# sag2021/ndsm

Hardware: AMD Instinct MI355X
Metric: fine-grid LUP/s (RB-GS smoother updates per second of V-cycle time, fp64) (higher is better)
Workload: dtype f64; 1 GPU; 512^3 vector-potential Ax component, one V-cycle + convergence metric per step (ms=5, 8 grids), config[2] of BASELINE.json; global_points=134217728, parallelism=single GPU

## Files before the change

ndsm_amd/csrc/smooth.hip:

```cpp
#include "common.hpp"

namespace ndsm {
void fused_metric_accumulate(bool on);
int launch_rbgs3_fused(const ndsmk_grid &g, const double *u, double *uout, const double *rhs, int max_sweeps,
                       bool force, int *sweeps_done, double *rout, int *res_done, const double *prev, int *met_done,
                       const ndsmk_xfer *px, const double *uc);
int fetch_fused_metric(double *h_out2);
int launch_mean_shift(double *u, int64_t n);
}

namespace {

__device__ __forceinline__ size_t lin3(int i, int j, int k, int nx, int ny) {
  return (size_t)i + (size_t)nx * ((size_t)j + (size_t)ny * (size_t)k);
}

__global__ __launch_bounds__(256) void rbgs3_color(double *__restrict__ u, const double *__restrict__ rhs,
                                                  ndsmk_grid g, int par) {
  const int nx = g.n[0], ny = g.n[1], nz = g.n[2];
  const int j = g.lb[1] + blockIdx.y * blockDim.y + threadIdx.y;
  const int k = g.lb[2] + blockIdx.z;
  if (j > g.ub[1]) return;
  const int kg = k + g.k0;
  const int i0 = g.lb[0] + ((((g.lb[0] + j + kg) & 1) != par) ? 1 : 0);
  const int i = i0 + 2 * (blockIdx.x * blockDim.x + threadIdx.x);
  if (i > g.ub[0]) return;
  int xl = i - 1, xh = i + 1, yl = j - 1, yh = j + 1, zl = k - 1, zh = k + 1;
  if (xl < 0) xl = 1;
  if (xh > nx - 1) xh = nx - 2;
  if (yl < 0) yl = 1;
  if (yh > ny - 1) yh = ny - 2;
  if (kg - 1 < 0) zl = k + 1;
  if (kg + 1 > g.nzg - 1) zh = k - 1;
  (void)nz;
  const double unew = (u[lin3(xh, j, k, nx, ny)] + u[lin3(xl, j, k, nx, ny)]) * g.w[0] +
                      (u[lin3(i, yh, k, nx, ny)] + u[lin3(i, yl, k, nx, ny)]) * g.w[1] +
                      (u[lin3(i, j, zh, nx, ny)] + u[lin3(i, j, zl, nx, ny)]) * g.w[2] -
                      (rhs ? rhs[lin3(i, j, k, nx, ny)] : 0.0);
  u[lin3(i, j, k, nx, ny)] = g.w1 * unew;
}

__global__ __launch_bounds__(1024) void rbgs3_small(double *__restrict__ u_g, const double *__restrict__ rhs_g,
                                                    ndsmk_grid g, int nsweeps) {
  __shared__ double u[4096], rhs[4096];
  const int nx = g.n[0], ny = g.n[1];
  const int n = nx * ny * g.n[2];
  for (int p = threadIdx.x; p < n; p += blockDim.x) {
    u[p] = u_g[p];
    rhs[p] = rhs_g ? rhs_g[p] : 0.0;
  }
  __syncthreads();
  const int mx = g.ub[0] - g.lb[0] + 1, my = g.ub[1] - g.lb[1] + 1, mz = g.ub[2] - g.lb[2] + 1;
  const int half = (mx + 1) / 2;
  const int total = half * my * mz;
  for (int sw = 0; sw < nsweeps; ++sw) {
    for (int pass = 0; pass < 2; ++pass) {
      const int par = (g.first_par + pass) & 1;
      for (int p = threadIdx.x; p < total; p += blockDim.x) {
        const int t = p % half, j = g.lb[1] + (p / half) % my, k = g.lb[2] + p / (half * my);
        const int i0 = g.lb[0] + ((((g.lb[0] + j + k) & 1) != par) ? 1 : 0);
        const int i = i0 + 2 * t;
        if (i > g.ub[0]) continue;
        int xl = i - 1, xh = i + 1, yl = j - 1, yh = j + 1, zl = k - 1, zh = k + 1;
        if (xl < 0) xl = 1;
        if (xh > nx - 1) xh = nx - 2;
        if (yl < 0) yl = 1;
        if (yh > ny - 1) yh = ny - 2;
        if (zl < 0) zl = 1;
        if (zh > g.n[2] - 1) zh = g.n[2] - 2;
        const double unew = (u[lin3(xh, j, k, nx, ny)] + u[lin3(xl, j, k, nx, ny)]) * g.w[0] +
                            (u[lin3(i, yh, k, nx, ny)] + u[lin3(i, yl, k, nx, ny)]) * g.w[1] +
                            (u[lin3(i, j, zh, nx, ny)] + u[lin3(i, j, zl, nx, ny)]) * g.w[2] -
                            rhs[lin3(i, j, k, nx, ny)];
        u[lin3(i, j, k, nx, ny)] = g.w1 * unew;
      }
      __syncthreads();
    }
  }
  for (int p = threadIdx.x; p < n; p += blockDim.x) u_g[p] = u[p];
}

__global__ __launch_bounds__(1024) void rbgs2_small(double *__restrict__ u_g, const double *__restrict__ rhs_g,
                                                    ndsmk_grid g, int nsweeps) {
  __shared__ double u[4096], rhs[4096];
  __shared__ double red[16];
  const int nx = g.n[0], ny = g.n[1];
  const int n = nx * ny;
  for (int p = threadIdx.x; p < n; p += blockDim.x) {
    u[p] = u_g[p];
    rhs[p] = rhs_g ? rhs_g[p] : 0.0;
  }
  __syncthreads();
  const int mx = g.ub[0] - g.lb[0] + 1, my = g.ub[1] - g.lb[1] + 1;
  const int half = (mx + 1) / 2;
  const int total = half * my;
  for (int sw = 0; sw < nsweeps; ++sw) {
    for (int pass = 0; pass < 2; ++pass) {
      const int par = (g.first_par + pass) & 1;
      for (int p = threadIdx.x; p < total; p += blockDim.x) {
        const int t = p % half, j = g.lb[1] + p / half;
        const int i0 = g.lb[0] + ((((g.lb[0] + j) & 1) != par) ? 1 : 0);
        const int i = i0 + 2 * t;
        if (i > g.ub[0]) continue;
        const int xl = (i == 0) ? 1 : (i == nx - 1 ? nx - 2 : i - 1);
        const int xh = (i == 0) ? 1 : (i == nx - 1 ? nx - 2 : i + 1);
        const int yl = (j == 0) ? 1 : (j == ny - 1 ? ny - 2 : j - 1);
        const int yh = (j == 0) ? 1 : (j == ny - 1 ? ny - 2 : j + 1);
        double un = 0.0;
        un = un + u[xl + nx * j] * g.w[0] + u[xh + nx * j] * g.w[0];
        un = un + u[i + nx * yl] * g.w[1] + u[i + nx * yh] * g.w[1];
        u[i + nx * j] = (un - rhs[i + nx * j]) * g.w1;
      }
      __syncthreads();
    }
    if (g.all_neumann) {
      double sm = 0.0;
      for (int p = threadIdx.x; p < n; p += blockDim.x) sm = sm + u[p];
      for (int o = 32; o > 0; o >>= 1) sm = sm + __shfl_down(sm, o, 64);
      if ((threadIdx.x & 63) == 0) red[threadIdx.x >> 6] = sm;
      __syncthreads();
      double tot = 0.0;
      for (int q = 0; q < 16; ++q) tot = tot + red[q];
      const double mean = tot / (double)n;
      for (int p = threadIdx.x; p < n; p += blockDim.x) u[p] = u[p] - mean;
      __syncthreads();
    }
  }
  for (int p = threadIdx.x; p < n; p += blockDim.x) u_g[p] = u[p];
}

constexpr int kMed2D = 19456;
__global__ __launch_bounds__(1024) void rbgs2_medium(double *__restrict__ u_g, const double *__restrict__ rhs_g,
                                                     ndsmk_grid g, int nsweeps) {
  extern __shared__ __attribute__((aligned(16))) double u[];
  __shared__ double red[16];
  constexpr int KQ = 8;
  const int nx = g.n[0], ny = g.n[1];
  const int n = nx * ny;
  for (int p = threadIdx.x; p < n; p += blockDim.x) u[p] = u_g[p];
  const int mx = g.ub[0] - g.lb[0] + 1, my = g.ub[1] - g.lb[1] + 1;
  const int half = (mx + 1) / 2;
  const int total = half * my;
  auto update = [&](int i, int j, double r) {
    const int xl = (i == 0) ? 1 : (i == nx - 1 ? nx - 2 : i - 1);
    const int xh = (i == 0) ? 1 : (i == nx - 1 ? nx - 2 : i + 1);
    const int yl = (j == 0) ? 1 : (j == ny - 1 ? ny - 2 : j - 1);
    const int yh = (j == 0) ? 1 : (j == ny - 1 ? ny - 2 : j + 1);
    double un = 0.0;
    un = un + u[xl + nx * j] * g.w[0] + u[xh + nx * j] * g.w[0];
    un = un + u[i + nx * yl] * g.w[1] + u[i + nx * yh] * g.w[1];
    u[i + nx * j] = (un - r) * g.w1;
  };
  auto point_of = [&](int p, int par, int &i, int &j) {
    const int t = p % half;
    j = g.lb[1] + p / half;
    i = g.lb[0] + ((((g.lb[0] + j) & 1) != par) ? 1 : 0) + 2 * t;
    return p < total && i <= g.ub[0];
  };
  int pij[2][KQ];
  double rr[2][KQ];
#pragma unroll
  for (int pass = 0; pass < 2; ++pass) {
#pragma unroll
    for (int q = 0; q < KQ; ++q) {
      int i, j;
      const bool have = point_of((int)threadIdx.x + 1024 * q, (g.first_par + pass) & 1, i, j);
      pij[pass][q] = have ? (i | (j << 16)) : -1;
      rr[pass][q] = (have && rhs_g) ? rhs_g[i + nx * j] : 0.0;
    }
  }
  __syncthreads();
  for (int sw = 0; sw < nsweeps; ++sw) {
#pragma unroll
    for (int pass = 0; pass < 2; ++pass) {
#pragma unroll
      for (int q = 0; q < KQ; ++q) {
        const int c = pij[pass][q];
        if (c >= 0) update(c & 0xffff, c >> 16, rr[pass][q]);
        if ((q & 3) == 3) __builtin_amdgcn_sched_barrier(0);
      }
      for (int p = (int)threadIdx.x + 1024 * KQ; p < total; p += 1024) {
        int i, j;
        if (point_of(p, (g.first_par + pass) & 1, i, j)) update(i, j, rhs_g ? rhs_g[i + nx * j] : 0.0);
      }
      __syncthreads();
    }
    if (g.all_neumann) {
      double sm = 0.0;
#pragma unroll 8
      for (int p = threadIdx.x; p < n; p += 1024) sm = sm + u[p];
      for (int o = 32; o > 0; o >>= 1) sm = sm + __shfl_down(sm, o, 64);
      if ((threadIdx.x & 63) == 0) red[threadIdx.x >> 6] = sm;
      __syncthreads();
      double tot = 0.0;
      for (int q = 0; q < 16; ++q) tot = tot + red[q];
      const double mean = tot / (double)n;
#pragma unroll 8
      for (int p = threadIdx.x; p < n; p += 1024) u[p] = u[p] - mean;
      __syncthreads();
    }
  }
  for (int p = threadIdx.x; p < n; p += blockDim.x) u_g[p] = u[p];
}

__global__ __launch_bounds__(256) void rbgs2_color(double *__restrict__ u, const double *__restrict__ rhs,
                                                  ndsmk_grid g, int par) {
  const int nx = g.n[0], ny = g.n[1];
  const int j = g.lb[1] + blockIdx.y * blockDim.y + threadIdx.y;
  if (j > g.ub[1]) return;
  const int i0 = g.lb[0] + ((((g.lb[0] + j) & 1) != par) ? 1 : 0);
  const int i = i0 + 2 * (blockIdx.x * blockDim.x + threadIdx.x);
  if (i > g.ub[0]) return;
  const int xl = (i == 0) ? 1 : (i == nx - 1 ? nx - 2 : i - 1);
  const int xh = (i == 0) ? 1 : (i == nx - 1 ? nx - 2 : i + 1);
  const int yl = (j == 0) ? 1 : (j == ny - 1 ? ny - 2 : j - 1);
  const int yh = (j == 0) ? 1 : (j == ny - 1 ? ny - 2 : j + 1);
  double un = 0.0;
  un = un + u[(size_t)xl + (size_t)nx * j] * g.w[0] + u[(size_t)xh + (size_t)nx * j] * g.w[0];
  un = un + u[(size_t)i + (size_t)nx * yl] * g.w[1] + u[(size_t)i + (size_t)nx * yh] * g.w[1];
  u[(size_t)i + (size_t)nx * j] = (un - (rhs ? rhs[(size_t)i + (size_t)nx * j] : 0.0)) * g.w1;
}

}

static int relax_impl(const ndsmk_grid *gp, double *const bufs[3], const double *keep, const double *rhs, int nsweeps,
                      int variant, int *where, double *rout, int *res_done, const double *prev, int *met_done,
                      const ndsmk_xfer *px = nullptr, const double *uc = nullptr) {
  NDSM_REQUIRE_READY();
  if (res_done) *res_done = 0;
  if (met_done) *met_done = 0;
  const ndsmk_grid g = *gp;
  NDSM_CHECK_ARG(g.ndim == 2 || g.ndim == 3);
  NDSM_CHECK_ARG(g.n[0] >= 2 && g.n[1] >= 2 && (g.ndim == 2 ? g.n[2] == 1 : g.n[2] >= 2));
  for (int d = 0; d < g.ndim; ++d) NDSM_CHECK_ARG(g.lb[d] >= 0 && g.ub[d] <= g.n[d] - 1);
  NDSM_CHECK_ARG(variant >= 0 && variant <= 2);
  NDSM_CHECK_ARG(g.ndim == 2 || (g.zown0 >= 0 && g.zown1 <= g.n[2] && g.zown0 < g.zown1));
  const int64_t npts = (int64_t)g.n[0] * g.n[1] * g.n[2];
  hipStream_t s = ndsm::stream();
  const int mx = g.ub[0] - g.lb[0] + 1, my = g.ub[1] - g.lb[1] + 1, mz = g.ub[2] - g.lb[2] + 1;
  int cur = 0;
  if (where) *where = 0;
  bool prol_pending = px != nullptr;
  if (prol_pending && (nsweeps <= 0 || mx <= 0 || my <= 0 || (g.ndim == 3 && mz <= 0))) {
    if (int rc = ndsmk_prolong_add(px, uc, bufs[0])) return rc;
    prol_pending = false;
  }
  if (mx <= 0 || my <= 0 || (g.ndim == 3 && mz <= 0)) return 0;
  auto in_place_ok = [&]() { return keep == nullptr || bufs[cur] != keep; };
  if (g.ndim == 3 && variant == 0 && !g.all_neumann && npts <= 4096 && g.k0 == 0 && g.zown0 == 0 &&
      g.zown1 == g.n[2] && nsweeps > 0) {
    NDSM_CHECK_ARG(in_place_ok());
    if (prol_pending) {
      if (int rc = ndsmk_prolong_add(px, uc, bufs[0])) return rc;
    }
    hipLaunchKernelGGL(rbgs3_small, dim3(1), dim3(1024), 0, s, bufs[0], rhs, g, nsweeps);
    NDSM_LAUNCH_CHECK();
    return 0;
  }
  if (g.ndim == 2 && variant == 0 && npts <= 4096 && nsweeps > 0) {
    NDSM_CHECK_ARG(in_place_ok());
    if (prol_pending) {
      if (int rc = ndsmk_prolong_add(px, uc, bufs[0])) return rc;
    }
    hipLaunchKernelGGL(rbgs2_small, dim3(1), dim3(1024), 0, s, bufs[0], rhs, g, nsweeps);
    NDSM_LAUNCH_CHECK();
    return 0;
  }
  if (g.ndim == 2 && variant == 0 && npts <= kMed2D && nsweeps > 0) {
    NDSM_CHECK_ARG(in_place_ok());
    if (prol_pending) {
      if (int rc = ndsmk_prolong_add(px, uc, bufs[0])) return rc;
    }
    static int attr_epoch = 0;
    if (ndsm::first_in_epoch(attr_epoch))
      NDSM_HIP(hipFuncSetAttribute(reinterpret_cast<const void *>(rbgs2_medium), hipFuncAttributeMaxDynamicSharedMemorySize,
                                   kMed2D * (int)sizeof(double)));
    hipLaunchKernelGGL(rbgs2_medium, dim3(1), dim3(1024), (size_t)npts * sizeof(double), s, bufs[0], rhs, g, nsweeps);
    NDSM_LAUNCH_CHECK();
    return 0;
  }
  for (int sw = 0; sw < nsweeps; ++sw) {
    double *u = bufs[cur];
    if (g.ndim == 3) {
      bool done = false;
      if (variant != 1) {
        int dst = -1;
        for (int c = 0; c < 3; ++c)
          if (c != cur && bufs[c] && bufs[c] != keep) {
            dst = c;
            break;
          }
        int ndone = 0;
        if (prol_pending) {
          int rc = ndsm::launch_rbgs3_fused(g, u, dst >= 0 ? bufs[dst] : nullptr, rhs, g.all_neumann ? 1 : nsweeps - sw,
                                            variant == 2, &ndone, nullptr, nullptr, nullptr, nullptr, px, uc);
          if (rc) return rc;
          if (ndone == 0) {
            NDSM_CHECK_ARG(in_place_ok());
            rc = ndsmk_prolong_add(px, uc, u);
            if (rc) return rc;
          }
          prol_pending = false;
        }
        int rc = ndone > 0 ? 0
                           : ndsm::launch_rbgs3_fused(g, u, dst >= 0 ? bufs[dst] : nullptr, rhs,
                                                      g.all_neumann ? 1 : nsweeps - sw, variant == 2, &ndone,
                                                      g.all_neumann ? nullptr : rout, res_done,
                                                      g.all_neumann ? nullptr : prev, met_done, nullptr, nullptr);
        if (rc) return rc;
        done = ndone > 0;
        if (done) {
          sw += ndone - 1;
          cur = dst;
          u = bufs[cur];
        }
        if (!done && variant == 2)
          return ndsm::fail(NDSMK_EARG, "fused smoother does not support this level shape", __FILE__, __LINE__);
      }
      if (!done && prol_pending) {
        NDSM_CHECK_ARG(in_place_ok());
        if (int rc = ndsmk_prolong_add(px, uc, u)) return rc;
        prol_pending = false;
      }
      if (!done) {
        if (g.zown0 != 0 || g.zown1 != g.n[2])
          return ndsm::fail(NDSMK_EARG, "z-slab levels need the fused smoother (nx even, >= 16 x 16 x 8 owned)", __FILE__,
                            __LINE__);
        NDSM_CHECK_ARG(in_place_ok());
        const int half = (mx + 1) / 2;
        dim3 block(64, 4, 1);
        dim3 grid((half + 63) / 64, (my + 3) / 4, mz);
        for (int pass = 0; pass < 2; ++pass) {
          hipLaunchKernelGGL(rbgs3_color, grid, block, 0, s, u, rhs, g, (g.first_par + pass) & 1);
          NDSM_LAUNCH_CHECK();
        }
      }
    } else {
      NDSM_CHECK_ARG(in_place_ok());
      if (prol_pending) {
        if (int rc = ndsmk_prolong_add(px, uc, u)) return rc;
        prol_pending = false;
      }
      const int half = (mx + 1) / 2;
      dim3 block(64, 4, 1);
      dim3 grid((half + 63) / 64, (my + 3) / 4, 1);
      for (int pass = 0; pass < 2; ++pass) {
        hipLaunchKernelGGL(rbgs2_color, grid, block, 0, s, u, rhs, g, (g.first_par + pass) & 1);
        NDSM_LAUNCH_CHECK();
      }
    }
    if (g.all_neumann) {
      int rc = ndsm::launch_mean_shift(u, npts);
      if (rc) return rc;
    }
  }
  if (cur != 0) {
    if (where) {
      *where = cur;
    } else {
      NDSM_HIP(hipMemcpyAsync(bufs[0], bufs[cur], sizeof(double) * (size_t)npts, hipMemcpyDeviceToDevice, s));
    }
  }
  return 0;
}

extern "C" int ndsmk_relax(const ndsmk_grid *gp, double *u, double *ualt, const double *rhs, int nsweeps,
                           int variant, int *result_in_alt) {
  double *const bufs[3] = {u, ualt, nullptr};
  return relax_impl(gp, bufs, nullptr, rhs, nsweeps, variant, result_in_alt, nullptr, nullptr, nullptr, nullptr);
}

extern "C" int ndsmk_relax_residual(const ndsmk_grid *gp, double *u, double *ualt, const double *rhs, double *r,
                                    int nsweeps, int variant, int *result_in_alt) {
  NDSM_CHECK_ARG(r != nullptr && result_in_alt != nullptr && (variant == 0 || variant == 2));
  int res_done = 0;
  double *const bufs[3] = {u, ualt, nullptr};
  int rc = relax_impl(gp, bufs, nullptr, rhs, nsweeps, variant, result_in_alt, r, &res_done, nullptr, nullptr);
  if (rc) return rc;
  if (!res_done) {
    if (variant == 2)
      return ndsm::fail(NDSMK_EARG, "fused sweep + residual does not cover this level", __FILE__, __LINE__);
    rc = ndsmk_residual(gp, *result_in_alt ? ualt : u, rhs, r);
  }
  return rc;
}

extern "C" int ndsmk_relax3(const ndsmk_grid *gp, double *u, double *a, double *b, const double *keep,
                            const double *rhs, int nsweeps, double *r, const double *prev, int *where,
                            int *met_done, const ndsmk_xfer *px, const double *uc) {
  NDSM_CHECK_ARG(where != nullptr && met_done != nullptr && u && a);
  int res_done = 0;
  double *const bufs[3] = {u, a, b};
  int rc = relax_impl(gp, bufs, keep, rhs, nsweeps, 0, where, r, &res_done, prev, met_done, px, uc);
  if (rc) return rc;
  if (r && !res_done) rc = ndsmk_residual(gp, bufs[*where], rhs, r);
  return rc;
}

extern "C" int ndsmk_fetch_fused_metric(double *h_out2) {
  NDSM_REQUIRE_READY();
  return ndsm::fetch_fused_metric(h_out2);
}

extern "C" int ndsmk_fused_window(const ndsmk_grid *gp, const double *u, double *uout, const double *rhs, int nsweeps,
                                  int z0, int z1, const ndsmk_xfer *px, const double *uc, const double *prev,
                                  int accumulate) {
  NDSM_REQUIRE_READY();
  ndsmk_grid g = *gp;
  NDSM_CHECK_ARG(g.ndim == 3 && (nsweeps == 1 || nsweeps == 2) && z0 >= g.zown0 && z1 <= g.zown1 && z0 < z1);
  NDSM_CHECK_ARG((!px || uc) && !(px && prev));
  g.zown0 = z0;
  g.zown1 = z1;
  int ndone = 0, met = 0;
  ndsm::fused_metric_accumulate(accumulate != 0);
  int rc = ndsm::launch_rbgs3_fused(g, u, uout, rhs, nsweeps, true, &ndone, nullptr, nullptr, prev, prev ? &met : nullptr,
                                    px, uc);
  ndsm::fused_metric_accumulate(false);
  if (rc) return rc;
  if (ndone != nsweeps || (prev && !met))
    return ndsm::fail(NDSMK_EARG, "fused smoother: this window / sweep count is not covered", __FILE__, __LINE__);
  return 0;
}

extern "C" int ndsmk_fused_window_res(const ndsmk_grid *gp, const double *u, double *uout, const double *rhs, double *rout,
                                      int z0, int z1) {
  NDSM_REQUIRE_READY();
  ndsmk_grid g = *gp;
  NDSM_CHECK_ARG(g.ndim == 3 && rout && z0 >= g.zown0 && z1 <= g.zown1 && z0 < z1);
  g.zown0 = z0;
  g.zown1 = z1;
  int ndone = 0, res = 0;
  int rc = ndsm::launch_rbgs3_fused(g, u, uout, rhs, 1, true, &ndone, rout, &res, nullptr, nullptr, nullptr, nullptr);
  if (rc) return rc;
  if (ndone != 1 || !res)
    return ndsm::fail(NDSMK_EARG, "fused sweep + residual: this window is not covered", __FILE__, __LINE__);
  return 0;
}

extern "C" int ndsmk_fused_metric_ok(const ndsmk_grid *gp) { return (gp->ndim == 3 && !gp->all_neumann) ? 1 : 0; }

extern "C" int ndsmk_fused_prolong_ok(const ndsmk_grid *gp, const double *rhs, int nsweeps) {
  return (gp->ndim == 3 && (!rhs || nsweeps == 1) && (nsweeps == 1 || nsweeps == 2) && !gp->all_neumann) ? 1 : 0;
}
```

Measured before the change: 265.0 billion LUP/s.

## Add shared-memory temporal-blocked RB-GS smoother for small and mid-size 3D levels

Adds a new kernel that loads a 3D tile with a halo of 2*S cells into shared memory and performs up to two red-black sweeps (four half-sweeps) inside it, using overlapping halos so that each cell is updated only where its dependency depth allows. The kernel is used as a fallback after the fused smoother on levels below 512K points, or as the first choice below an env-configurable threshold. The aim is to cut kernel launches and global memory round-trips on coarse levels, at the cost of redundant halo computation.

```diff
diff --git a/ndsm_amd/csrc/smooth.hip b/ndsm_amd/csrc/smooth.hip
--- a/ndsm_amd/csrc/smooth.hip
+++ b/ndsm_amd/csrc/smooth.hip
@@ -5,6 +5,9 @@
 int launch_rbgs3_fused(const ndsmk_grid &g, const double *u, double *uout, const double *rhs, int max_sweeps,
                        bool force, int *sweeps_done, double *rout, int *res_done, const double *prev, int *met_done,
                        const ndsmk_xfer *px, const double *uc);
+int launch_rbgs3_block(const ndsmk_grid &g, const double *u, double *uout, const double *rhs, int max_sweeps,
+                       int *sweeps_done);
+int64_t block_smoother_first_below();
 int fetch_fused_metric(double *h_out2);
 int launch_mean_shift(double *u, int64_t n);
 }
@@ -291,9 +294,15 @@
             break;
           }
         int ndone = 0;
+        const int64_t blk_first_below = ndsm::block_smoother_first_below();
+        const bool blk = variant == 0 && dst >= 0 && !g.all_neumann && npts > 4096 && g.k0 == 0 && g.zown0 == 0 &&
+                         g.zown1 == g.n[2] && (npts < (int64_t)512 * 1024 || npts < blk_first_below);
+        const bool blk_first = blk && npts < blk_first_below;
         if (prol_pending) {
-          int rc = ndsm::launch_rbgs3_fused(g, u, dst >= 0 ? bufs[dst] : nullptr, rhs, g.all_neumann ? 1 : nsweeps - sw,
-                                            variant == 2, &ndone, nullptr, nullptr, nullptr, nullptr, px, uc);
+          int rc = blk_first ? 0
+                             : ndsm::launch_rbgs3_fused(g, u, dst >= 0 ? bufs[dst] : nullptr, rhs,
+                                                        g.all_neumann ? 1 : nsweeps - sw, variant == 2, &ndone, nullptr,
+                                                        nullptr, nullptr, nullptr, px, uc);
           if (rc) return rc;
           if (ndone == 0) {
             NDSM_CHECK_ARG(in_place_ok());
@@ -302,12 +311,17 @@
           }
           prol_pending = false;
         }
-        int rc = ndone > 0 ? 0
-                           : ndsm::launch_rbgs3_fused(g, u, dst >= 0 ? bufs[dst] : nullptr, rhs,
-                                                      g.all_neumann ? 1 : nsweeps - sw, variant == 2, &ndone,
-                                                      g.all_neumann ? nullptr : rout, res_done,
-                                                      g.all_neumann ? nullptr : prev, met_done, nullptr, nullptr);
+        int rc = ndone > 0 || blk_first
+                     ? 0
+                     : ndsm::launch_rbgs3_fused(g, u, dst >= 0 ? bufs[dst] : nullptr, rhs,
+                                                g.all_neumann ? 1 : nsweeps - sw, variant == 2, &ndone,
+                                                g.all_neumann ? nullptr : rout, res_done,
+                                                g.all_neumann ? nullptr : prev, met_done, nullptr, nullptr);
         if (rc) return rc;
+        if (ndone == 0 && blk) {
+          rc = ndsm::launch_rbgs3_block(g, u, bufs[dst], rhs, nsweeps - sw, &ndone);
+          if (rc) return rc;
+        }
         done = ndone > 0;
         if (done) {
           sw += ndone - 1;
diff --git a/ndsm_amd/csrc/smooth_block.hip b/ndsm_amd/csrc/smooth_block.hip
--- /dev/null
+++ b/ndsm_amd/csrc/smooth_block.hip
@@ -0,0 +1,151 @@
+#include <cstdlib>
+#include <cstring>
+
+#include "common.hpp"
+
+namespace {
+
+constexpr int kNT = 1024;
+constexpr int kFar = 15;
+
+template <int S, int BX, int BY, int BZ>
+__global__ __launch_bounds__(kNT) void rbgs3_block_k(const double *__restrict__ u, double *__restrict__ uout,
+                                                     const double *__restrict__ rhs, ndsmk_grid g) {
+  constexpr int R = 2 * S;
+  constexpr int LX = BX + 2 * R, LY = BY + 2 * R, LZ = BZ + 2 * R;
+  constexpr int NL = LX * LY * LZ;
+  constexpr int HX = LX / 2;
+  constexpr int NSLOT = HX * LY * LZ;
+  constexpr int NIT = (NSLOT + kNT - 1) / kNT;
+  constexpr int NLD = (NL + kNT - 1) / kNT;
+  static_assert(LX % 2 == 0 && NL * 8 < 65536, "tile does not fit");
+  __shared__ double t[NL];
+  const int nx = g.n[0], ny = g.n[1], nz = g.n[2];
+  const int tid = threadIdx.x;
+  const int ox = (int)blockIdx.x * BX - R, oy = (int)blockIdx.y * BY - R, oz = (int)blockIdx.z * BZ - R;
+  auto at = [&](int i, int j, int k) { return (size_t)i + (size_t)nx * ((size_t)j + (size_t)ny * (size_t)k); };
+
+  double v[NLD];
+#pragma unroll
+  for (int q = 0; q < NLD; ++q) {
+    const int p = tid + kNT * q;
+    const int i = ox + p % LX, j = oy + (p / LX) % LY, k = oz + p / (LX * LY);
+    v[q] = (p < NL && i >= 0 && i < nx && j >= 0 && j < ny && k >= 0 && k < nz) ? u[at(i, j, k)] : 0.0;
+  }
+
+  auto depth = [](int c, int o, int L, int n) {
+    const int lo = o <= 0 ? kFar : c - o;
+    const int hi = o + L - 1 >= n - 1 ? kFar : o + L - 1 - c;
+    return lo < hi ? lo : hi;
+  };
+  int code[2][NIT];
+  double rr[2][NIT];
+#pragma unroll
+  for (int q = 0; q < NIT; ++q) {
+    const int p = tid + kNT * q;
+    const int jl = (p / HX) % LY, kl = p / (HX * LY);
+    const int j = oy + jl, k = oz + kl;
+    const bool row = p < NSLOT && j >= g.lb[1] && j <= g.ub[1] && k >= g.lb[2] && k <= g.ub[2];
+    const int dy = depth(j, oy, LY, ny), dz = depth(k, oz, LZ, nz);
+    const int dyz = dy < dz ? dy : dz;
+    const int fyz = (j == 0 ? 4 : 0) | (j == ny - 1 ? 8 : 0) | (k == 0 ? 16 : 0) | (k == nz - 1 ? 32 : 0);
+    const int first = (g.first_par + j + k + ox) & 1;
+#pragma unroll
+    for (int c = 0; c < 2; ++c) {
+      const int il = 2 * (p % HX) + (first ^ c);
+      const int i = ox + il;
+      const int dx = depth(i, ox, LX, nx);
+      const int d = dx < dyz ? dx : dyz;
+      const bool ok = row && i >= g.lb[0] && i <= g.ub[0] && d >= c + 1;
+      const int fl = fyz | (i == 0 ? 1 : 0) | (i == nx - 1 ? 2 : 0);
+      code[c][q] = ok ? ((il + LX * (jl + LY * kl)) | (d << 16) | (fl << 20)) : -1;
+      rr[c][q] = (ok && rhs) ? rhs[at(i, j, k)] : 0.0;
+    }
+  }
+#pragma unroll
+  for (int q = 0; q < NLD; ++q) {
+    const int p = tid + kNT * q;
+    if (p < NL) t[p] = v[q];
+  }
+  __syncthreads();
+
+#pragma unroll
+  for (int h = 0; h < 2 * S; ++h) {
+#pragma unroll
+    for (int q = 0; q < NIT; ++q) {
+      const int cd = code[h & 1][q];
+      if (cd >= 0 && ((cd >> 16) & 15) >= h + 1) {
+        const int p = cd & 0xffff;
+        const int xl = (cd & (1 << 20)) ? p + 1 : p - 1, xh = (cd & (2 << 20)) ? p - 1 : p + 1;
+        const int yl = (cd & (4 << 20)) ? p + LX : p - LX, yh = (cd & (8 << 20)) ? p - LX : p + LX;
+        const int zl = (cd & (16 << 20)) ? p + LX * LY : p - LX * LY, zh = (cd & (32 << 20)) ? p - LX * LY : p + LX * LY;
+        const double unew = (t[xh] + t[xl]) * g.w[0] + (t[yh] + t[yl]) * g.w[1] + (t[zh] + t[zl]) * g.w[2] - rr[h & 1][q];
+        t[p] = g.w1 * unew;
+      }
+    }
+    __syncthreads();
+  }
+
+  const int bx0 = ox + R, by0 = oy + R, bz0 = oz + R;
+  for (int p = tid; p < BX * BY * BZ; p += kNT) {
+    const int il = p % BX, jl = (p / BX) % BY, kl = p / (BX * BY);
+    const int i = bx0 + il, j = by0 + jl, k = bz0 + kl;
+    if (i < nx && j < ny && k < nz) uout[at(i, j, k)] = t[(il + R) + LX * ((jl + R) + LY * (kl + R))];
+  }
+}
+
+template <int S, int BZ>
+int launch_block(const ndsmk_grid &g, const double *u, double *uout, const double *rhs) {
+  constexpr int BX = 16, BY = 8;
+  const dim3 grid((g.n[0] + BX - 1) / BX, (g.n[1] + BY - 1) / BY, (g.n[2] + BZ - 1) / BZ);
+  hipLaunchKernelGGL((rbgs3_block_k<S, BX, BY, BZ>), grid, dim3(kNT), 0, ndsm::stream(), u, uout, rhs, g);
+  NDSM_LAUNCH_CHECK();
+  return 0;
+}
+
+const int64_t *block_cfg() {
+  static int64_t cfg[2] = {-1, 0};
+  if (cfg[0] < 0) {
+    cfg[0] = 0;
+    const char *e = std::getenv("NDSM_BLOCK_CFG");
+    for (int i = 0; e && i < 2; ++i) {
+      cfg[i] = std::atoll(e);
+      e = std::strchr(e, ',');
+      if (e) ++e;
+    }
+  }
+  return cfg;
+}
+
+}
+
+namespace ndsm {
+
+bool block_smoother_on() {
+  static const bool on = std::getenv("NDSM_HIP_NO_BLOCK") == nullptr;
+  return on;
+}
+
+int64_t block_smoother_first_below() { return block_cfg()[1]; }
+
+int launch_rbgs3_block(const ndsmk_grid &g, const double *u, double *uout, const double *rhs, int max_sweeps,
+                       int *sweeps_done) {
+  *sweeps_done = 0;
+  if (!block_smoother_on() || !uout || uout == u || g.ndim != 3 || g.all_neumann || max_sweeps < 1) return 0;
+  if (g.k0 != 0 || g.zown0 != 0 || g.zown1 != g.n[2] || g.nzg != g.n[2]) return 0;
+  if (g.n[0] < 2 || g.n[1] < 2 || g.n[2] < 2) return 0;
+  const int64_t gx = (g.n[0] + 15) / 16, gy = (g.n[1] + 7) / 8, gz8 = (g.n[2] + 7) / 8, gz4 = (g.n[2] + 3) / 4;
+  if (gy > 65535 || gz4 > 65535) return 0;
+  const int64_t bz = block_cfg()[0];
+  const bool low = bz == 4 || (bz != 8 && gx * gy * gz8 < 64);
+  int rc;
+  if (max_sweeps >= 2)
+    rc = low ? launch_block<2, 4>(g, u, uout, rhs) : launch_block<2, 8>(g, u, uout, rhs);
+  else
+    rc = low ? launch_block<1, 4>(g, u, uout, rhs) : launch_block<1, 8>(g, u, uout, rhs);
+  if (rc) return rc;
+  *sweeps_done = max_sweeps >= 2 ? 2 : 1;
+  return 0;
+}
+
+}
```

Measured after the change: 268.4 billion LUP/s, median of 6. +1.3%, better.
